# swiss-territorial-data-lab/proj-roadsurf

Hardware: AMD Instinct MI355X
Metric: tiles_per_sec_512x512x3 (higher is better)
Workload: dtype f16 hi + lo operand planes (22 significand bits, 3 MFMA products per product) / f32 accumulate; 1 GPU; Mask R-CNN R50-FPN inference, batch 16 of 512x512 3-band tiles per GPU (BASELINE configs[1]), 800x800 network input; seeded synthetic weights, saturated: 1000 proposals and 100 detections per tile; batch_per_gpu=16, lanes=2, lane_streams=independent, num_classes=2, weights=random

## Files before the change

### include/rs_engine.h

```cpp
#ifndef RS_ENGINE_H
#define RS_ENGINE_H

#include <stddef.h>
#include <stdint.h>

#ifdef __cplusplus
extern "C" {
#endif

#define RS_ABI_VERSION 1
#define RS_SPEC_MAX_LEVELS 5
#define RS_SPEC_MAX_ANCHORS 8
#define RS_NUM_PHASES 3
#define RS_MASK_SIDE 28
#define RS_MAX_CLASSES 80
#define RS_TRAIN_MAX_CLASSES 8

typedef struct rs_spec {
  int32_t struct_size;
  int32_t in_channels;
  int32_t flip_channels;
  float pixel_mean[4];
  float pixel_std[4];
  int32_t min_size_test;
// ... 100 lines not shown
                     const void* w1p, const float* b1, void* t1n, const void* x0, const void* wsc, int n, int h, int w, int width,
                     void* stream);

int rs_op_bneck_tail_split(const void* t1, int64_t t1_lo, const void* w2, const float* s2, const float* b2, const void* w3p, const float* s3,
                           const float* b3, const void* x, int64_t x_lo, void* out, int64_t out_lo, const void* w1p, const float* s1,
                           const float* b1, void* t1n, int64_t t1n_lo, const void* x0, int64_t x0_lo, int n, int h, int w, int width,
                           void* stream);

int rs_op_mask_overlap(const uint8_t* det_masks, int n_det, const uint8_t* label_masks, int n_labels, int h, int w, int32_t* inter,
                       int32_t* label_area, void* stream);
int rs_engine_label_overlap(rs_engine* e, int tile, const uint8_t* label_masks_dev, int n_labels, int32_t* inter_dev, int32_t* label_area_dev);

int rs_op_conv_variant(int m, int cin, int k, int cout, int cin2, int deconv2x, int out_f32, int* stages_out);

int rs_debug_set_conv_probe(void* buffer);

int rs_op_set_saturation_counter(void* dev_u64);

int rs_op_conv2d_split(const void* in, int64_t in_lo, const void* w, int64_t w_lo, const float* wscale, const float* bias, void* out, int64_t out_lo,
                       const void* residual, int64_t res_lo, const void* upsample_add, int64_t up_lo,
                       int n, int hi, int wi, int cin, int in_halo, int kh, int kw, int stride, int pad, int cout, int kpad,
                       int out_halo, int relu, int out_f32, int deconv2x, int variant, void* stream);

int rs_op_conv2d_dual(const void* in, const void* in2, const void* w, const float* bias, void* out,
                      int n, int hi, int wi, int cin, int in_halo, int kh, int kw, int stride, int pad,
                      int h2, int w2, int cin2, int in2_halo, int stride2,
                      int cout, int kpad, int out_halo, int relu, int variant, void* stream);

int rs_op_conv2d_dgrad(const void* dy, const void* w_t, void* dx, const void* res, const float* res32, const void* mask,
                       const void* down, int n, int hi, int wi, int cin, int ho, int wo, int cout, int kh, int kw, int stride,
                       int pad, int kpad, int halo, int variant, void* stream);

int rs_op_conv2d_wgrad(const void* dy, const void* in, float* grad, const float* scale, int n, int hi, int wi, int cin,
                       int in_halo, int kh, int kw, int stride, int pad, int cout, int kpad, int dy_halo, int splits,
                       void* stream);
int rs_op_conv2d_wgrad_f32(const void* dy, const void* in, float* grad, const float* scale, int n, int hi, int wi, int cin,
                       int in_halo, int kh, int kw, int stride, int pad, int cout, int kpad, int dy_halo, int splits,
                       void* stream);

int rs_op_nms(const float* boxes, const int32_t* counts, const uint8_t* valid, uint8_t* keep,
              int segments, int cap, float thresh, void* stream);
int rs_op_batched_nms(const float* boxes, const int32_t* counts, const uint8_t* valid, uint8_t* keep, int images,
                      int segments_per_image, int cap, float thresh, int rule, void* stream);
int rs_op_batched_nms_decision(const float* boxes, const int32_t* counts, const uint8_t* valid, uint8_t* keep, int images,
                               int segments_per_image, int cap, float thresh, int rule, int32_t* rule_out, float* unit_out, void* stream);

// ... 99 lines not shown
```

### proj_roadsurf_amd/csrc/common.h

```cpp
#pragma once
#include <hip/hip_runtime.h>
#include <stdint.h>
#include <stdio.h>

typedef _Float16 half_t;
typedef _Float16 half4 __attribute__((ext_vector_type(4)));
typedef _Float16 half8 __attribute__((ext_vector_type(8)));
typedef float f32x4 __attribute__((ext_vector_type(4)));

#define RS_OK 0
#define RS_ERR_ARG -1
#define RS_ERR_HIP -2
#define RS_ERR_BLOB -3
#define RS_ERR_UNSUPPORTED -4

void rs_set_error(const char* fmt, ...);

#define RS_HIP(expr)                                                                       \
  do {                                                                                     \
    hipError_t _e = (expr);                                                                \
    if (_e != hipSuccess) {                                                                \
      rs_set_error("%s:%d: %s -> %s", __FILE__, __LINE__, #expr, hipGetErrorString(_e));   \
      return RS_ERR_HIP;                                                                   \
    }                                                                                      \
// ... 116 lines not shown
  const half_t* mask;
  int out_stride;
  long long* probe;
  int persist;
  int stages;
  const half_t* head_w;
  const float* head_b;
  float* head_out;
  int nseg;
  int seg_tiles;
  int tail_tiles;
  int split;
  long long in_lo, w_lo, out_lo, res_lo, up_lo, in2_lo;
  const float* wscale;
  long long head_w_lo;
  const float* head_scale;
  ConvSeg seg[RS_MAX_SEGS];
  unsigned long long* sat;
};

int launch_conv(const ConvParams& p, hipStream_t stream, int force_variant , int use_glds);
int conv_choose_variant(ConvParams& p, int force_variant, int use_glds);
extern thread_local int g_last_conv_variant;

struct StemPoolParams {
  const half_t* in;
  const half_t* wf;
  const float* bias;
  half_t* out;
  int N, in_Hp, in_Wp;
  int Hc, Wc;
  int Hq, Wq;
  unsigned long long* sat;
};
int launch_stem_pool(const StemPoolParams& p, hipStream_t stream);
struct StemPoolSplitParams {
  const half_t* in; long long in_lo;
  const half_t* wf;
  const float* wscale;
  const float* bias;
  half_t* out; long long out_lo;
  int N, in_Hp, in_Wp;
  int Hc, Wc;
  int Hq, Wq;
  unsigned long long* sat;
};
// ... 93 lines not shown
```

### proj_roadsurf_amd/csrc/conv_deep.hip

```cpp
#include "common.h"

namespace {

constexpr int BN = 256, NT = 512, MI = 4, WCH = 4;
constexpr int ASTAGE = 256 * 128, WSTAGE = BN * 128;
constexpr int W_BASE = 3 * ASTAGE;
constexpr int LDS_BYTES = 3 * ASTAGE + 2 * WSTAGE;

__device__ __forceinline__ void glds16(const half_t* g, char* lds_wave_base) {
  __builtin_amdgcn_global_load_lds((const __attribute__((address_space(1))) void*)g,
                                   (__attribute__((address_space(3))) void*)lds_wave_base, 16, 0, 0);
}

template <int DBG, bool TRAIN, int NJ, bool SPLIT>
__device__ __forceinline__ void conv_deep_tile(const ConvParams& p, char* smem, const half_t* g_in, const half_t* g_w, const float* g_bias, void* g_out,
                                               float* g_head_out, const int Ho, const int Wo, const int in_Hp, const int in_Wp, const int out_Hp, const int out_Wp,
                                               const int M, const int m0, const int n0, const int q, const long long in_lo, const long long out_lo,
                                               const float* g_wscale) {
  constexpr int APS = (NJ + 1) / 2;
  constexpr int WPX = NJ * 16;
  const int tid = threadIdx.x;
  const int lane = tid & 63;
  const int wave = __builtin_amdgcn_readfirstlane(tid >> 6);
  const int wpx = wave / WCH, wch = wave % WCH;
  (void)q;

  const int lrow = lane >> 3, lchk = lane & 7;
  const half_t* aptr[APS];
  const half_t* wptr[4];
  unsigned aoffb[APS], woffb[4];
#pragma unroll
  for (int ps = 0; ps < APS; ++ps) {
    int m = m0 + ps * 64 + wave * 8 + lrow;
    if (m >= M) m = M - 1;
    const int x = m % Wo;
    const int t = m / Wo;
    const int y = t % Ho;
// ... 270 lines not shown
  }

#ifdef RS_CLOCK_PROBE
  if (p.probe && tid == 0) {
    p.probe[2 * q] = (long long)(__builtin_amdgcn_s_memtime() - pr_t0);
    p.probe[2 * q + 1] = (long long)(__builtin_amdgcn_s_memrealtime() - pr_r0);
  }
#endif
  const int crow = n0 + wch * 64 + fq * 16;
  float bias[16];
#pragma unroll
  for (int i = 0; i < MI; ++i) {
    const f32x4 b4 = *(const f32x4*)(g_bias + crow + i * 4);
    bias[i * 4 + 0] = b4[0]; bias[i * 4 + 1] = b4[1]; bias[i * 4 + 2] = b4[2]; bias[i * 4 + 3] = b4[3];
  }
  float wsc[SPLIT ? 16 : 1];
  if constexpr (SPLIT) {
#pragma unroll
    for (int i = 0; i < MI; ++i) {
      const f32x4 s4 = *(const f32x4*)(g_wscale + crow + i * 4);
      wsc[i * 4 + 0] = s4[0]; wsc[i * 4 + 1] = s4[1]; wsc[i * 4 + 2] = s4[2]; wsc[i * 4 + 3] = s4[3];
    }
  }
  unsigned satc = 0;
  if (!TRAIN && SPLIT && p.head_w) {
    const half_t* hw = p.head_w + (long long)fi * 256 + wch * 64 + fq * 8;
    const half8 ha0 = *(const half8*)hw, ha1 = *(const half8*)(hw + 32);
    const half8 hl0 = *(const half8*)(hw + p.head_w_lo), hl1 = *(const half8*)(hw + p.head_w_lo + 32);
    f32x4 hacc[NJ];
#pragma unroll
    for (int j = 0; j < NJ; ++j) {
      half8 b0, b1, l0, l1;
      const bool mv = m0 + wpx * WPX + j * 16 + fi < M;
      unsigned sath = 0;
#pragma unroll
      for (int i = 0; i < MI; ++i)
#pragma unroll
        for (int r = 0; r < 4; ++r) {
          float f = acc[i][j][r] * wsc[i * 4 + r] + bias[i * 4 + r];
          if (p.relu) f = f > 0.f ? f : 0.f;
          sath += mv ? rs_sat_bad(f) : 0u;
          f = f > 65504.f ? 65504.f : (f < -65504.f ? -65504.f : f);
          const half_t h = (half_t)f;
          const half_t l = (half_t)(f - (float)h);
          if (i < 2) { b0[i * 4 + r] = h; l0[i * 4 + r] = l; } else { b1[(i - 2) * 4 + r] = h; l1[(i - 2) * 4 + r] = l; }
        }
// ... 228 lines not shown
  }
  if (p.nseg) {
    int t0 = 0;
#pragma unroll
    for (int i = 0; i < RS_MAX_SEGS; ++i)
      if (i < p.nseg && L >= p.seg[i].tile0) {
        g_in = p.seg[i].in; g_w = p.seg[i].w; g_bias = p.seg[i].bias; g_out = p.seg[i].out; g_head_out = p.seg[i].head_out;
        Ho = p.seg[i].Ho; Wo = p.seg[i].Wo; in_Hp = p.seg[i].in_Hp; in_Wp = p.seg[i].in_Wp;
        out_Hp = p.seg[i].out_Hp; out_Wp = p.seg[i].out_Wp; M = p.seg[i].M; t0 = p.seg[i].tile0;
        if constexpr (SPLIT) { in_lo = p.seg[i].in_lo; out_lo = p.seg[i].out_lo; g_wscale = p.seg[i].wscale; }
      }
    L -= t0;
  }
  const int n0 = (L % tiles_n) * BN;
  const int m0 = (L / tiles_n) * BM;
  if (half < 0 || NJF != 8) {
    conv_deep_tile<DBG, TRAIN, NJF, SPLIT>(p, smem, g_in, g_w, g_bias, g_out, g_head_out, Ho, Wo, in_Hp, in_Wp, out_Hp, out_Wp, M, m0, n0, q, in_lo, out_lo, g_wscale);
  } else {
    if (m0 + half * (BM / 2) >= M) return;
    conv_deep_tile<DBG, TRAIN, NJF == 8 ? 4 : NJF, SPLIT>(p, smem, g_in, g_w, g_bias, g_out, g_head_out, Ho, Wo, in_Hp, in_Wp, out_Hp, out_Wp, M, m0 + half * (BM / 2), n0, q, in_lo, out_lo, g_wscale);
  }
}

}

int rs_device_cu_count() {
  static int ncu[64] = {0};
  int dev = 0;
  if (hipGetDevice(&dev) != hipSuccess || dev < 0 || dev >= 64) return 256;
  if (!ncu[dev]) {
    int n = 0;
    if (hipDeviceGetAttribute(&n, hipDeviceAttributeMultiprocessorCount, dev) != hipSuccess || n <= 0) n = 256;
    ncu[dev] = n;
  }
  return ncu[dev];
}

static int deep_tail_tiles(long long tiles) {
  const int ncu = rs_device_cu_count();
  if (!rs_debug().deep_tail) return 0;
  const int r = (int)(tiles % ncu);
  return (r > 0 && 2 * r <= ncu) ? r : 0;
}

static int no_scratch(const void* kernel, const char* what) {
  hipFuncAttributes a;
// ... 3 lines not shown
  return RS_OK;
}

template <int NJF>
static int launch_deep_nj(ConvParams& p, hipStream_t stream) {
  static bool done = false;
  if (!done) {
    RS_HIP(hipFuncSetAttribute((const void*)conv_deep_kernel<0, false, NJF>, hipFuncAttributeMaxDynamicSharedMemorySize, LDS_BYTES));
    if constexpr (NJF >= 5) RS_HIP(hipFuncSetAttribute((const void*)conv_deep_kernel<0, false, NJF, true>, hipFuncAttributeMaxDynamicSharedMemorySize, LDS_BYTES));
    { int rc = no_scratch((const void*)conv_deep_kernel<0, false, NJF>, "conv_deep_kernel"); if (rc) return rc; }
    if constexpr (NJF >= 5) { int rc = no_scratch((const void*)conv_deep_kernel<0, false, NJF, true>, "conv_deep_kernel (split operands)"); if (rc) return rc; }
    done = true;
  }
  const long long nblk = (long long)(p.Cout / BN) * cdiv(p.M, 32 * NJF);
  RS_CHECK(nblk < (1ll << 30), RS_ERR_ARG, "conv_deep: grid too large");
  p.tail_tiles = 0;
  if (p.split) {
    if constexpr (NJF >= 5) hipLaunchKernelGGL((conv_deep_kernel<0, false, NJF, true>), dim3((unsigned)nblk), dim3(NT), LDS_BYTES, stream, p);
    else RS_CHECK(false, RS_ERR_UNSUPPORTED, "conv_deep: the split-operand mode has the 160 .. 256-pixel tiles only");
    RS_HIP(hipGetLastError());
    return RS_OK;
  }
  hipLaunchKernelGGL((conv_deep_kernel<0, false, NJF>), dim3((unsigned)nblk), dim3(NT), LDS_BYTES, stream, p);
  RS_HIP(hipGetLastError());
  return RS_OK;
}

int launch_conv_deep(const ConvParams& p0, hipStream_t stream, int tile_px) {
  ConvParams p = p0;
  p.nseg = 0;
  RS_CHECK(p.mode == 0 && !p.in2 && p.Cin % 64 == 0 && p.Cout % BN == 0 && p.M > 0, RS_ERR_ARG,
           "conv_deep: unsupported shape (mode %d, Cin %d, Cout %d)", p.mode, p.Cin, p.Cout);
  RS_CHECK(!p.head_w || (p.Cout == BN && p.head_b && p.head_out && !p.res && !p.up && !p.down && !p.res32 && !p.mask), RS_ERR_ARG,
           "conv_deep: the fused head needs Cout == 256, its bias and output, and no other epilogue option");
  RS_CHECK(p.out_stride <= 1, RS_ERR_UNSUPPORTED, "conv_deep: no strided scatter");
  RS_CHECK(!p.split || (p.wscale && (!p.head_w || p.head_scale) && !p.down && !p.res32 && !p.mask), RS_ERR_UNSUPPORTED, "conv_deep: the split-operand mode needs the row scales (the fused head's too) and has no training epilogue");
  if (p.split) {
    const long long in_px = (long long)cdiv(p.M, p.Ho * p.Wo) * p.in_Hp * p.in_Wp;
    RS_CHECK((p.in_lo + in_px * p.in_Cs) * 2 < (1ll << 32) && (p.w_lo + (long long)p.Cout * p.Kpad) * 2 < (1ll << 32), RS_ERR_UNSUPPORTED,
             "conv_deep: split-operand tensor of more than 4 GB (input %lld elements per plane)", in_px * p.in_Cs);
  }
  if (tile_px != 256) {
    RS_CHECK(tile_px >= 64 && tile_px <= 224 && tile_px % 32 == 0 && !p.down && !p.res32 && !p.mask, RS_ERR_ARG,
             "conv_deep: tile height %d (256, or 64 .. 224 in steps of 32 without training epilogue options)", tile_px);
    switch (tile_px / 32) {
      case 2: return launch_deep_nj<2>(p, stream);
// ... 96 lines not shown
```

### proj_roadsurf_amd/csrc/conv_igemm.hip

```cpp
#include "common.h"

namespace {

template <int WPX, int WCH, int MI, int NJ>
struct Tile {
  static constexpr int NW = WPX * WCH;
  static constexpr int NT = NW * 64;
  static constexpr int BM = WPX * NJ * 16;
  static constexpr int BN = WCH * MI * 16;
  static constexpr int STAGE = (BM + BN) * 128;
  static constexpr int LDS = 2 * STAGE + 1024;
};

__device__ __forceinline__ void glds16(const half_t* g, char* lds_wave_base) {
  __builtin_amdgcn_global_load_lds((const __attribute__((address_space(1))) void*)g,
                                   (__attribute__((address_space(3))) void*)lds_wave_base, 16, 0, 0);
}

template <int WPX, int WCH, int MI, int NJ, bool SMALLC, bool GLDS, bool PERSIST, bool TRAIN = false, bool SPLIT = false>
__global__ __launch_bounds__(WPX* WCH * 64) void conv_igemm_kernel(const ConvParams p) {
  using T = Tile<WPX, WCH, MI, NJ>;
  constexpr int NW = T::NW, BM = T::BM, BN = T::BN;
  constexpr int PA = BM / (NW * 8);
  constexpr int PW = (BN + NW * 8 - 1) / (NW * 8);
// ... 541 lines not shown

int launch_conv(const ConvParams& p_in, hipStream_t stream, int force_variant, int use_glds) {
  if (use_glds < 0) {
    RS_CHECK(!p_in.in2, RS_ERR_UNSUPPORTED, "conv: the fp32 kernel has no second K source");
    g_last_conv_variant = -1;
    return launch_conv_f32(p_in, stream, use_glds == -2, force_variant);
  }
  ConvParams p = p_in;
  const int nk2 = p.in2 ? (p.Cin2 >> 6) : 0;
  const bool train_opts = p.down || p.res32 || p.mask || p.out_stride > 1;
  RS_CHECK(p.M > 0, RS_ERR_ARG, "conv: M=%d", p.M);
  RS_CHECK(p.Kpad % 64 == 0, RS_ERR_ARG, "conv: Kpad %d not a multiple of 64", p.Kpad);
  const bool smallc = p.Cin < 64;
  if (smallc) {
    RS_CHECK((p.Cin == 8 || p.Cin == 4) && p.koff != nullptr, RS_ERR_ARG, "conv: small-Cin path needs Cin 4 or 8 and a koff table");
  } else {
    RS_CHECK(p.Cin % 64 == 0, RS_ERR_ARG, "conv: Cin %d not a multiple of 64", p.Cin);
    RS_CHECK(p.KH * p.KW * p.Cin + nk2 * 64 <= p.Kpad, RS_ERR_ARG, "conv: K exceeds Kpad");
  }
  if (p.in2) RS_CHECK(!smallc && p.mode == 0 && p.Cin2 % 64 == 0 && p.Cin2 > 0 && p.stride2 >= 1, RS_ERR_ARG, "conv: bad second K source (Cin2 %d)", p.Cin2);
  const int rows = p.Cout * (p.mode != 0 ? 4 : 1);
  int v = conv_choose_variant(p, force_variant, use_glds);
  if (v == 22 && p.mode == 2 && !conv_wreg_ok(p)) v = 14;
  RS_CHECK(!(train_opts && (p.mode != 0 || (v == 12 && p.out_stride > 1) || (v >= 15 && v <= 20))), RS_ERR_UNSUPPORTED, "conv: training epilogue options need mode 0 (and no scatter on conv_deep)");
  if (v == 22 || v == 23 || v == 25 || v == 26) {
    RS_CHECK(conv_wreg_ok(p) && !train_opts, RS_ERR_UNSUPPORTED, "conv: variant %d takes 1x1 / Cin 256 / Cout %% 256 == 0 inference layers only", v);
    g_last_conv_variant = v;
    return launch_conv_wreg(p, stream, v == 23 ? 8 : (v == 25 ? 2 : (v == 26 ? 4 : 0)));
  }
  if (v == 12 || (v >= 15 && v <= 20)) {
    RS_CHECK(!p.in2, RS_ERR_UNSUPPORTED, "conv: variant %d has no second K source", v);
    g_last_conv_variant = v;
    return launch_conv_deep(p, stream, v == 12 ? 256 : (v <= 17 ? 160 + 32 * (v - 15) : 64 + 32 * (v - 18)));
  }
  RS_CHECK(!(p.mode != 0 && p.Cout % 128 != 0), RS_ERR_ARG, "deconv needs Cout %% 128 == 0");
  RS_CHECK(!(p.mode == 2 && !(p.dot_w && p.dot_cls && p.dot_slot && p.dot_out && (v == 0 || v == 10 || v == 14))), RS_ERR_ARG, "fused mask predictor needs its pointers and the 128x128, 64x256 or 128x256 tile");
  g_last_conv_variant = smallc ? 5 : v;
  if (smallc) {
    RS_CHECK(v == 1, RS_ERR_ARG, "conv: small-Cin path is built for the 256x64 tile only (Cout=%d)", p.Cout);
    if (rs_debug().stem_small_tile) return launch_variant<4, 1, 4, 2, true, false>(p, stream, use_glds);
    return launch_variant<4, 1, 4, 4, true, false>(p, stream, use_glds);
  }
  switch (v) {
    case 0:
      RS_CHECK(rows % 128 == 0, RS_ERR_ARG, "conv: variant 0 needs Cout %% 128 == 0");
      return launch_variant<2, 2, 4, 4, false, true>(p, stream, use_glds);
    case 1:
      RS_CHECK(rows % 64 == 0, RS_ERR_ARG, "conv: variant 1 needs Cout %% 64 == 0");
      return launch_variant<4, 1, 4, 4, false, true>(p, stream, use_glds);
    case 2:
      RS_CHECK(rows % 16 == 0 && p.out_f32, RS_ERR_ARG, "conv: variant 2 is the 16-channel-tile fp32-out head kernel");
// ... 28 lines not shown
```

### proj_roadsurf_amd/csrc/detect.h

```cpp
#pragma once
#include "common.h"

#define RS_MAX_LEVELS 5
#define RS_MAX_ANCHORS 8

struct RpnParams {
  const float* head[RS_MAX_LEVELS];
  uint32_t* keys[RS_MAX_LEVELS];
  int H[RS_MAX_LEVELS], W[RS_MAX_LEVELS], stride[RS_MAX_LEVELS];
  float base[RS_MAX_LEVELS][RS_MAX_ANCHORS][4];
  float offset;
  int L, A, N, cs;
  int topk;
  float img_h, img_w;
  const float* img_hw;
  float wx, wy, ww, wh, scale_clamp, min_size;
  float* cand_boxes;
  float* cand_scores;
  uint8_t* cand_valid;
  int* cand_count;
  int* cand_index;
  int debug;
  int cand_cap;
};
// ... 79 lines not shown
  int K, cap, dets_per_image;
  float scale_x, scale_y, out_w, out_h;
  float* det_boxes_net;
  float* det_boxes;
  float* det_scores;
  int* det_classes;
  int* det_roi;
  int* det_count;
  unsigned long long* part_keys;
  int* part_count;
};

struct MaskPredictParams {
  const half_t* in;
  const float* w;
  const float* b;
  const int* slot_list;
  const int* det_classes;
  const int* n_entries;
  float* out;
  int S;
  int f32;
  long long in_lo;
};

struct PasteParams {
  const float* probs;
  const float* det_boxes;
  const int* slot_list;
  const int* n_entries;
  uint8_t* out;
  int S, out_h, out_w;
  float threshold;
};

struct CropParams {
  const float* det_boxes;
  const int* det_count;
  const uint8_t* masks;
  int n, D, h, w, Wb;
  int* rects;
  unsigned int* offsets;
  unsigned long long* total;
  uint8_t* data;
};
int launch_mask_crops(const CropParams& p, hipStream_t s);
// ... 13 lines not shown
```

### proj_roadsurf_amd/csrc/detect_kernels.hip

```cpp
#include "detect.h"

namespace {

__device__ __forceinline__ uint32_t fkey(float f) {
  f = f + 0.0f;
  const uint32_t u = __float_as_uint(f);
  return (u & 0x80000000u) ? ~u : (u | 0x80000000u);
}
__device__ __forceinline__ float fkey_inv(uint32_t k) {
  const uint32_t u = (k & 0x80000000u) ? (k & 0x7fffffffu) : ~k;
  return __uint_as_float(u);
}

template <int T>
__device__ void bitonic_sort_desc(unsigned long long* s, int n, int tid) {
  for (int k = 2; k <= n; k <<= 1) {
    for (int j = k >> 1; j > 0; j >>= 1) {
      for (int i = tid; i < n; i += T) {
        const int ixj = i ^ j;
        if (ixj > i) {
          const unsigned long long a = s[i], b = s[ixj];
          const bool desc = (i & k) == 0;
          if (desc ? (a < b) : (a > b)) { s[i] = b; s[ixj] = a; }
        }
// ... 1457 lines not shown
    const half_t* x = p.in + pix * 256 + sub * 16;
    const half8 a = *(const half8*)x, b = *(const half8*)(x + 8);
#pragma unroll
    for (int i = 0; i < 8; ++i) { xv[i] = (float)a[i]; xv[8 + i] = (float)b[i]; }
  }
  float s = 0.f;
#pragma unroll
  for (int i = 0; i < 16; ++i) s += xv[i] * w[i];
  s += __shfl_xor(s, 8, 16);
  s += __shfl_xor(s, 4, 16);
  s += __shfl_xor(s, 2, 16);
  s += __shfl_xor(s, 1, 16);
  if (sub == 0) {
    const float logit = s + p.b[cls];
    const float prob = rs_fdiv(1.f, 1.f + expf(-logit));
    p.out[(long long)slot * SS + (pix - (long long)entry * SS)] = prob;
  }
}

__global__ __launch_bounds__(256) void mask_sigmoid_kernel(const MaskPredictParams p) {
  const int total = *p.n_entries;
  const int SS = p.S * p.S;
  const long long gid = (long long)blockIdx.x * 256 + threadIdx.x;
  if (gid >= (long long)total * SS) return;
  const int entry = (int)(gid / SS);
  const int slot = p.slot_list[entry];
  float* o = p.out + (long long)slot * SS + (gid - (long long)entry * SS);
  const float logit = *o + p.b[p.det_classes[slot]];
  *o = rs_fdiv(1.f, 1.f + expf(-logit));
}

__global__ __launch_bounds__(256) void paste_masks_kernel(const PasteParams p) {
  const int total = *p.n_entries;
  const int Wb = (p.out_w + 7) >> 3;
  const int Ww = (Wb + 3) >> 2;
  const long long gid = (long long)blockIdx.x * 256 + threadIdx.x;
  const long long per = (long long)p.out_h * Ww;
  if (gid >= (long long)total * per) return;
  const int entry = (int)(gid / per);
  const int rem = (int)(gid - (long long)entry * per);
  const int y = rem / Ww, xw = rem - y * Ww;
  const int slot = p.slot_list[entry];
  const float* bx = p.det_boxes + (long long)slot * 4;
  const float x0 = bx[0], y0 = bx[1], x1 = bx[2], y1 = bx[3];
  const float* m = p.probs + (long long)slot * p.S * p.S;
  const int S = p.S;
  unsigned int word = 0;
// ... 273 lines not shown
```

### proj_roadsurf_amd/csrc/engine.hip

```cpp
#include <stdarg.h>
#include <string.h>

#include <cmath>
#include <functional>
#include <map>
#include <set>
#include <string>
#include <vector>

#include "../../include/rs_engine.h"
#include "detect.h"
#include "train.h"

static thread_local char g_err[1024] = "";
static bool g_trainer_unfused_shortcut = false;

static RsDebug g_debug;
static bool g_debug_loaded = false;
void rs_debug_reload() {
  RsDebug d;
  auto rd = [](const char* name, int* v) { const char* e = getenv(name); if (e && *e) *v = atoi(e); };
  rd("RS_CONV_SINGLE_STAGE_NK", &d.conv_single_stage_nk); rd("RS_CONV_PERSIST", &d.conv_persist); rd("RS_CONV_TUNED", &d.conv_tuned);
  rd("RS_CONV_DEEP", &d.conv_deep); rd("RS_CONV_WIDE_PX", &d.conv_wide_px); rd("RS_CONV_WREG", &d.conv_wreg); rd("RS_WREG_DBG", &d.wreg_dbg); rd("RS_ROI_BWD_ATOMIC", &d.roi_bwd_atomic); rd("RS_WREG_WAVES", &d.wreg_waves); rd("RS_STEM_SMALL_TILE", &d.stem_small_tile); rd("RS_DEEP_DBG", &d.deep_dbg);
  rd("RS_DECONV_VARIANT", &d.deconv_variant); rd("RS_FUSE_MASK_PREDICTOR", &d.fuse_mask_predictor); rd("RS_SIDE_STREAM", &d.side_stream);
  rd("RS_NARROW_ROIALIGN", &d.narrow_roialign); rd("RS_USE_GLDS", &d.use_glds); rd("RS_FUSE_SHORTCUT", &d.fuse_shortcut); rd("RS_MERGE_LEVELS", &d.merge_levels); rd("RS_FUSE_RPN_HEADS", &d.fuse_rpn_heads); rd("RS_DEEP_TAIL", &d.deep_tail); rd("RS_DEEP_TILE_PX", &d.deep_tile_px); rd("RS_FUSE_BNECK", &d.fuse_bneck); rd("RS_FUSE_STEM", &d.fuse_stem);
  rd("RS_USE_GRAPH", &d.use_graph); rd("RS_GRAPH_SMALL", &d.graph_small); rd("RS_TRAIN_ROI_SIDE", &d.train_roi_side);
  rd("RS_TRAIN_SIDE", &d.train_side); rd("RS_WGRAD_TARGET", &d.wgrad_target); rd("RS_WGRAD_CB", &d.wgrad_cb);
  rd("RS_SELECT_DEBUG", &d.select_debug); rd("RS_NMS_DEBUG", &d.nms_debug); rd("RS_ROI_WINDOW", &d.roi_window); rd("RS_ROI_ORDER", &d.roi_order);
// ... 1026 lines not shown
    RS_CHECK(dw && db && wrows(dw) == 1024, RS_ERR_BLOB, "deconv weights missing / wrong rows");
    RS_CHECK(pw && pb && pw->dtype == DT_F32, RS_ERR_BLOB, "mask predictor weights missing");
    const bool fuse = f32 ? false : rs_debug().fuse_mask_predictor != 0;
    ConvParams dp;
    memset(&dp, 0, sizeof dp);
    if ((rc = set_split(&dp, "roi_heads.mask_head.deconv", dw, &curm, nullptr, nullptr, nullptr, nullptr))) return rc;
    dp.in = curm.p; dp.w = (const half_t*)dw->dev; dp.bias = (const float*)db->dev;
    dp.Ho = MR; dp.Wo = MR; dp.in_Hp = curm.Hp(); dp.in_Wp = curm.Wp(); dp.in_Cs = 256; dp.in_off = 1; dp.stride = 1; dp.KH = dp.KW = 1;
    dp.Cin = 256; dp.Kpad = (int)dw->dims[1]; dp.Cout = 256; dp.out_Hp = 2 * MR; dp.out_Wp = 2 * MR; dp.out_Cs = 256; dp.out_pad = 0; dp.relu = 1;
    dp.m_count = det_total; dp.m_mul = MR * MR;
    const int per_roi = MR * MR;
    if (fuse) {
      dp.mode = 2; dp.out = nullptr;
      dp.dot_w = (const float*)pw->dev; dp.dot_cls = det_classes; dp.dot_slot = slot_list; dp.dot_out = mask_probs;
      dp.dot_k = (int)pw->dims[0];
      const int glds = use_glds, Dc = D;
      const bool sp = split;
      float* probs = mask_probs;
      const size_t zero_per_tile = (size_t)D * RS_MASK_SIDE * RS_MASK_SIDE * 4;
      Stage st;
      st.name = "mask.deconv_predict";
      st.flops_per_image = 2.0 * D * per_roi * 256 * 1024 + 2.0 * D * RS_MASK_SIDE * RS_MASK_SIDE * 256;
      st.bytes_per_image = (double)D * per_roi * 256 * 2 * (split ? 2 : 1) + (double)D * RS_MASK_SIDE * RS_MASK_SIDE * 4;
      st.fn = [dp, per_roi, Dc, glds, probs, zero_per_tile, sp](int n, hipStream_t s) mutable {
        RS_HIP(hipMemsetAsync(probs, 0, zero_per_tile * n, s));
        dp.M = n * Dc * per_roi;
        const int dv = rs_debug().deconv_variant;
        return launch_conv(dp, s, (dv == 22 && (sp || !(rs_debug().conv_wreg && glds > 0))) ? 14 : dv, glds);
      };
      stages.push_back(st);
      MaskPredictParams mp;
      mp.f32 = 0;
      mp.in = nullptr; mp.w = nullptr; mp.b = (const float*)pb->dev; mp.slot_list = slot_list; mp.det_classes = det_classes;
      mp.n_entries = det_total; mp.out = mask_probs; mp.S = RS_MASK_SIDE;
      Stage st2;
      st2.name = "mask.bias_sigmoid";
      st2.fn = [mp, Dc](int n, hipStream_t s) { return launch_mask_sigmoid(mp, n * Dc, s); };
      stages.push_back(st2);
    } else {
      Act dec;
      if ((rc = new_act(&dec, "mask_deconv", R, 2 * MR, 2 * MR, 256, 0))) return rc;
      dp.mode = 1; dp.out = dec.p; dp.out_lo = dec.lo;
      {
        const int glds = use_glds, Dc = D;
        Stage st;
        st.name = "mask.deconv";
        st.flops_per_image = 2.0 * D * per_roi * 256 * 1024;
        st.bytes_per_image = (double)D * per_roi * 256 * 2 * 5;
        dp.sat = sat_slot();
        st.fn = [dp, per_roi, Dc, glds](int n, hipStream_t s) mutable { dp.M = n * Dc * per_roi; return launch_conv(dp, s, -1, glds); };
        stages.push_back(st);
      }
      MaskPredictParams mp;
      mp.in = dec.p; mp.w = (const float*)pw->dev; mp.b = (const float*)pb->dev; mp.slot_list = slot_list; mp.det_classes = det_classes;
      mp.n_entries = det_total; mp.out = mask_probs; mp.S = RS_MASK_SIDE; mp.f32 = f32 ? 1 : (split ? 2 : 0); mp.in_lo = dec.lo;
      Stage st;
      st.name = "mask.predict_sigmoid";
      st.bytes_per_image = (double)D * RS_MASK_SIDE * RS_MASK_SIDE * (256 * 2 + 4);
      const int Dc = D;
      st.fn = [mp, Dc](int n, hipStream_t s) { return launch_mask_predict(mp, n * Dc, s); };
      stages.push_back(st);
    }
    const int Wb = (tile_w + 7) / 8;
    if ((rc = alloc((void**)&masks, (size_t)R * tile_h * Wb))) return rc;
    reg("masks", masks, DT_U8, {NB, D, tile_h, Wb}, 0);
    if ((rc = alloc((void**)&crop_data, (size_t)R * tile_h * Wb))) return rc;
    if ((rc = alloc((void**)&crop_rects, (size_t)R * 16))) return rc;
    if ((rc = alloc((void**)&crop_offsets, (size_t)R * 4))) return rc;
    if ((rc = alloc((void**)&crop_total, 16))) return rc;
    {
      PasteParams pm;
      pm.probs = mask_probs; pm.det_boxes = det_boxes; pm.slot_list = slot_list; pm.n_entries = det_total; pm.out = masks;
      pm.S = RS_MASK_SIDE; pm.out_h = tile_h; pm.out_w = tile_w; pm.threshold = S.mask_threshold;
      Stage st;
      st.name = "mask.paste";
      st.bytes_per_image = (double)D * tile_h * Wb;
// ... 447 lines not shown
  const Stage& s = e->stages[i];
  if (name_out) { strncpy(name_out, s.name.c_str(), 95); name_out[95] = 0; }
  if (ms_total) *ms_total = s.ms_total;
  if (calls) *calls = s.calls;
  if (flops) *flops = s.last_flops;
  if (bytes) *bytes = s.last_bytes;
  return RS_OK;
}

int rs_engine_stage_kernel(rs_engine* e, int i, char* name_out) {
  RS_CHECK(e && i >= 0 && i < (int)e->stages.size() && name_out, RS_ERR_ARG, "stage index");
  static const char* names[] = {"conv_igemm_kernel<2,2,4,4> 128x128", "conv_igemm_kernel<4,1,4,4> 256x64", "conv_igemm_kernel<4,1,1,4> 256x16 f32-out",
                                "conv_igemm_kernel<4,2,4,4> 256x128", "conv_igemm_kernel<2,4,4,8> 256x256", "conv_igemm_kernel<4,1,4,4,smallC> 256x64 stem",
                                "(retired)",
                                "conv_igemm_kernel<2,2,4,2> 64x128", "conv_igemm_kernel<4,1,4,2> 128x64", "conv_igemm_kernel<2,2,4,1> 32x128",
                                "conv_igemm_kernel<2,4,4,2> 64x256", "(retired)",
                                "conv_deep_kernel 256x256 (3 activation + 2 weight LDS stages)",
                                "bneck_tail_kernel 128 px (conv2 + conv3 + next conv1 chained through registers)",
                                "conv_igemm_kernel<2,4,4,4> 128x256",
                                "conv_deep_kernel 160x256", "conv_deep_kernel 192x256", "conv_deep_kernel 224x256",
                                "conv_deep_kernel 64x256", "conv_deep_kernel 96x256", "conv_deep_kernel 128x256",
                                "stem_pool_kernel (conv 7x7 s2 + ReLU + max-pool 3x3 s2, 8x8 pooled pixels per workgroup)",
                                "conv1x1_wreg_kernel 32 px x 256 ch (persistent, weights in registers, operand tiles by LDS-DMA, two workgroups per CU)",
                                "bneck_tail_split_kernel 128 px (conv2 + conv3 + next conv1 chained through registers)"};
  const int v = e->stages[i].variant;
  const char* s = v == -1 ? "conv_f32_mfma_kernel" : (v >= 0 && v <= 23 ? names[v] : "");
  if (e->split && v >= 0 && v <= 23) {
    snprintf(name_out, 96, "%.62s [split: hi+lo planes, 3 MFMA blocks]", s);
    return RS_OK;
  }
  strncpy(name_out, s, 95);
  name_out[95] = 0;
  return RS_OK;
}

int rs_engine_stage_variant(rs_engine* e, int i) {
  if (!e || i < 0 || i >= (int)e->stages.size()) return -2;
  return e->stages[i].variant;
}

int rs_op_conv_variant(int m, int cin, int k, int cout, int cin2, int deconv2x, int out_f32, int* stages_out) {
  ConvParams p;
  memset(&p, 0, sizeof p);
  p.M = m; p.Cin = cin; p.KH = p.KW = k; p.Cout = cout; p.mode = deconv2x ? 1 : 0; p.out_f32 = out_f32;
  p.stride = 1; p.in_Cs = cin; p.out_Cs = cout;
  p.Kpad = (k * k * (cin < 64 ? 8 : cin) + cin2 + 63) / 64 * 64;
  if (cin < 64 && k == 7) p.Kpad = 256;
  static const half_t dummy = (half_t)0;
  if (cin2 > 0) { p.in2 = &dummy; p.Cin2 = cin2; }
  const int v = conv_choose_variant(p, -1, 1);
// ... 81 lines not shown
  }
  return rc;
}

int rs_debug_set_conv_probe(void* buffer) { g_conv_probe = (long long*)buffer; return RS_OK; }
int rs_op_set_saturation_counter(void* dev_u64) { g_op_sat = (unsigned long long*)dev_u64; return RS_OK; }

int rs_op_conv2d(const void* in, const void* w, const float* bias, void* out, const void* residual, const void* upsample_add,
                 int n, int hi, int wi, int cin, int in_halo, int kh, int kw, int stride, int pad, int cout, int kpad,
                 int out_halo, int relu, int out_f32, int deconv2x, int variant, int use_glds, void* stream) {
  return op_conv2d(in, w, bias, out, residual, upsample_add, n, hi, wi, cin, in_halo, kh, kw, stride, pad, cout, kpad, out_halo,
                   relu, out_f32, deconv2x, variant, use_glds, stream, nullptr, 0, 0, 0, 0, 1);
}

int rs_op_conv2d_split(const void* in, int64_t in_lo, const void* w, int64_t w_lo, const float* wscale, const float* bias, void* out, int64_t out_lo,
                       const void* residual, int64_t res_lo, const void* upsample_add, int64_t up_lo,
                       int n, int hi, int wi, int cin, int in_halo, int kh, int kw, int stride, int pad, int cout, int kpad,
                       int out_halo, int relu, int out_f32, int deconv2x, int variant, void* stream) {
  SplitArgs sa = {in_lo, w_lo, out_lo, res_lo, up_lo, wscale};
  return op_conv2d(in, w, bias, out, residual, upsample_add, n, hi, wi, cin, in_halo, kh, kw, stride, pad, cout, kpad, out_halo,
                   relu, out_f32, deconv2x, variant, 1, stream, nullptr, 0, 0, 0, 0, 1, &sa);
}

int rs_op_conv2d_dual(const void* in, const void* in2, const void* w, const float* bias, void* out,
                      int n, int hi, int wi, int cin, int in_halo, int kh, int kw, int stride, int pad,
                      int h2, int w2, int cin2, int in2_halo, int stride2,
                      int cout, int kpad, int out_halo, int relu, int variant, void* stream) {
  RS_CHECK(in2, RS_ERR_ARG, "null argument");
  return op_conv2d(in, w, bias, out, nullptr, nullptr, n, hi, wi, cin, in_halo, kh, kw, stride, pad, cout, kpad, out_halo,
                   relu, 0, 0, variant, 1, stream, in2, h2, w2, cin2, in2_halo, stride2);
}

int rs_op_bneck_tail(const void* t1, const void* w2, const float* b2, const void* w3p, const float* b3, const void* x, void* out,
                     const void* w1p, const float* b1, void* t1n, const void* x0, const void* wsc, int n, int h, int w, int width, void* stream) {
  RS_CHECK(t1 && w2 && b2 && w3p && b3 && out && n > 0 && h > 0 && w > 0, RS_ERR_ARG, "bad argument");
  RS_CHECK(width == 64 || width == 128, RS_ERR_UNSUPPORTED, "bneck_tail: bottleneck width %d (64 or 128)", width);
  BneckParams p;
  memset(&p, 0, sizeof p);
  p.t1 = (const half_t*)t1; p.w2 = (const half_t*)w2; p.b2 = b2; p.w3p = (const half_t*)w3p; p.b3 = b3; p.x = (const half_t*)x; p.out = (half_t*)out;
  p.w1p = (const half_t*)w1p; p.b1 = b1; p.t1n = (half_t*)t1n; p.x0 = (const half_t*)x0; p.wsc = (const half_t*)wsc;
  p.M = n * h * w; p.H = h; p.W = w; p.Hp = h + 2; p.Wp = w + 2; p.CB = width / 64;
  p.sat = g_op_sat;
  return launch_bneck_tail(p, (hipStream_t)stream);
}

int rs_op_bneck_tail_split(const void* t1, int64_t t1_lo, const void* w2, const float* s2, const float* b2, const void* w3p, const float* s3, const float* b3,
// ... 281 lines not shown
```

### proj_roadsurf_amd/engine.py

```python
from __future__ import annotations

import ctypes as C
import weakref
import math
import os
import time
from typing import Any, Dict, Iterator, List, Optional, Sequence, Tuple

import numpy as np

from .spec import BATCHED_NMS_MODES, EngineSpec
from .weights import pack_weights

_LIB: Optional[C.CDLL] = None
LIB_PATH = os.environ.get("RS_ENGINE_LIB") or os.path.join(os.path.dirname(os.path.abspath(__file__)), "librs_engine.so")
MAX_LEVELS, MAX_ANCHORS, MASK_SIDE = 5, 8, 28
DT_NP = {1: np.float16, 2: np.float32, 3: np.int32, 4: np.uint8, 5: np.float16}
DT_SPLIT16 = 5


class RsError(RuntimeError):
    pass


# ... 80 lines not shown
    lib.rs_engine_fetch_crops_async.argtypes = [vp, i32, C.POINTER(RsDets), C.POINTER(RsMaskCrops)]
    lib.rs_engine_fetch_crops_wait.argtypes = [vp, C.POINTER(RsMaskCrops)]
    lib.rs_engine_fetch.argtypes = [vp, i32, C.POINTER(RsDets)]
    lib.rs_engine_stream.argtypes = [vp]
    lib.rs_engine_stream.restype = vp
    lib.rs_engine_set_profiling.argtypes = [vp, i32]
    lib.rs_debug_run_stages_matching.argtypes = [vp, C.c_char_p, i32]
    lib.rs_engine_stage_count.argtypes = [vp]
    lib.rs_engine_saturation.argtypes = [vp, C.POINTER(C.c_int64), i32]
    lib.rs_op_set_saturation_counter.argtypes = [vp]
    lib.rs_engine_stage_info.argtypes = [vp, i32, C.c_char_p, C.POINTER(C.c_double), i32p, C.POINTER(C.c_double), C.POINTER(C.c_double)]
    lib.rs_engine_stage_kernel.argtypes = [vp, i32, C.c_char_p]
    lib.rs_engine_stage_variant.argtypes = [vp, i32]
    lib.rs_op_conv_variant.argtypes = [i32] * 7 + [i32p]
    lib.rs_engine_tensor.argtypes = [vp, C.c_char_p, C.POINTER(vp), i32p, i32p, C.POINTER(C.c_int64), i32p]
    lib.rs_engine_tensor_count.argtypes = [vp]
    lib.rs_engine_tensor_name.argtypes = [vp, i32, C.c_char_p]
    lib.rs_engine_net_shape.argtypes = [vp, i32p, i32p, i32p, i32p]
    lib.rs_op_conv2d.argtypes = [vp, vp, vp, vp, vp, vp] + [i32] * 17 + [vp]
    lib.rs_op_bneck_tail.argtypes = [vp] * 12 + [i32, i32, i32, i32, vp]
    lib.rs_op_conv2d_dual.argtypes = [vp, vp, vp, vp, vp] + [i32] * 19 + [vp]
    i64 = C.c_int64
    lib.rs_op_conv2d_split.argtypes = [vp, i64, vp, i64, vp, vp, vp, i64, vp, i64, vp, i64] + [i32] * 16 + [vp]
    lib.rs_op_bneck_tail_split.argtypes = [vp, i64, vp, vp, vp, vp, vp, vp, vp, i64, vp, i64, vp, vp, vp, vp, i64, vp, i64, i32, i32, i32, i32, vp]
    lib.rs_op_conv2d_dgrad.argtypes = [vp] * 7 + [i32] * 14 + [vp]
    lib.rs_op_conv2d_wgrad.argtypes = [vp, vp, vp, vp] + [i32] * 13 + [vp]
    lib.rs_op_nms.argtypes = [vp, vp, vp, vp, i32, i32, C.c_float, vp]
    lib.rs_op_batched_nms.argtypes = [vp, vp, vp, vp, i32, i32, i32, C.c_float, i32, vp]
    lib.rs_op_batched_nms_decision.argtypes = [vp, vp, vp, vp, i32, i32, i32, C.c_float, i32, vp, vp, vp]
    lib.rs_op_det_merge.argtypes = [vp] * 5 + [i32] * 4 + [C.c_float] * 4 + [vp] * 7
    lib.rs_spec_batched_nms.argtypes = [C.POINTER(RsSpec)]
    lib.rs_op_roi_align.argtypes = [C.POINTER(vp), i32p, i32p, f32p, i32, vp, i32, i32, i32, i32, vp, vp, vp]
    lib.rs_op_roi_align_bwd.argtypes = [C.POINTER(vp), i32p, i32p, f32p, i32, vp, i32, i32, i32, i32, vp, vp]
    f32 = C.c_float
    lib.rs_op_match.argtypes = [vp, i32, vp, vp, vp, vp, vp, vp, i32, i32, i32, f32, f32, i32, i32, i32, i32, vp]
    lib.rs_op_subsample.argtypes = [vp, vp, vp, i32, i32, i32, f32, i32, i32, C.c_uint32, vp]
    lib.rs_op_rpn_loss.argtypes = [vp] * 6 + [i32] * 6 + [f32, f32, vp]
    lib.rs_op_box_loss.argtypes = [vp] * 6 + [i32, i32, i32, f32, f32p, f32, vp]
    lib.rs_op_mask_loss.argtypes = [vp] * 5 + [i32, i32, i32, f32, vp]
    lib.rs_op_sgd_momentum.argtypes = [vp, vp, vp, C.c_int64, f32, f32, f32, f32, i32, vp]
    lib.rs_op_fold_weights.argtypes = [vp] * 4 + [i32] * 6 + [vp]
    lib.rs_resize_shape.argtypes = [i32, i32, i32, i32, i32p, i32p]
    lib.rs_resize_shape.restype = None
    lib.rs_resize_coeffs.argtypes = [i32, i32, i32p, i32p]
    i64p, f64p = C.POINTER(C.c_int64), C.POINTER(C.c_double)
    lib.rs_vectorize_masks.argtypes = [vp, i32, i32, i32, C.c_double, i32]
# ... 1041 lines not shown
```

Measured before the change: 918.1 tiles/s.

## Fuse split-operand mask deconv with per-class predictor dot in conv_deep kernel

Adds a DOT path to the conv_deep tile that applies scale, bias and ReLU to the deconv accumulators, dots them with the selected class's predictor weights, reduces across waves in LDS, and writes mask logits straight to their 2x-upsampled positions. This variant is now the default for the split-precision mask deconv. It also drops the full memset of the logits buffer; the sigmoid kernel instead zeroes only the unused detection slots. The intent is to avoid the slower variant-14 path plus the separate predictor pass and memset, at the cost of an extra LDS reduction and a barrier in the epilogue.

```diff
diff --git a/include/rs_engine.h b/include/rs_engine.h
--- a/include/rs_engine.h
+++ b/include/rs_engine.h
@@ -146,6 +146,10 @@
                        int n, int hi, int wi, int cin, int in_halo, int kh, int kw, int stride, int pad, int cout, int kpad,
                        int out_halo, int relu, int out_f32, int deconv2x, int variant, void* stream);
 
+int rs_op_deconv_predict_split(const void* in, int64_t in_lo, const void* w, int64_t w_lo, const float* wscale, const float* bias, const float* dot_w,
+                               int dot_k, const int* dot_cls, const int* dot_slot, const int* m_count, float* logits, int slots, int n, int h, int wd,
+                               int cin, int in_halo, int kpad, int variant, void* stream);
+
 int rs_op_conv2d_dual(const void* in, const void* in2, const void* w, const float* bias, void* out,
                       int n, int hi, int wi, int cin, int in_halo, int kh, int kw, int stride, int pad,
                       int h2, int w2, int cin2, int in2_halo, int stride2,
diff --git a/proj_roadsurf_amd/csrc/common.h b/proj_roadsurf_amd/csrc/common.h
--- a/proj_roadsurf_amd/csrc/common.h
+++ b/proj_roadsurf_amd/csrc/common.h
@@ -162,6 +162,8 @@
 int launch_conv(const ConvParams& p, hipStream_t stream, int force_variant , int use_glds);
 int conv_choose_variant(ConvParams& p, int force_variant, int use_glds);
 extern thread_local int g_last_conv_variant;
+bool conv_deep_dot_ok(const ConvParams& p);
+int launch_conv_deep_dot(const ConvParams& p, hipStream_t stream);
 
 struct StemPoolParams {
   const half_t* in;
diff --git a/proj_roadsurf_amd/csrc/conv_deep.hip b/proj_roadsurf_amd/csrc/conv_deep.hip
--- a/proj_roadsurf_amd/csrc/conv_deep.hip
+++ b/proj_roadsurf_amd/csrc/conv_deep.hip
@@ -12,7 +12,7 @@
                                    (__attribute__((address_space(3))) void*)lds_wave_base, 16, 0, 0);
 }
 
-template <int DBG, bool TRAIN, int NJ, bool SPLIT>
+template <int DBG, bool TRAIN, int NJ, bool SPLIT, bool DOT = false>
 __device__ __forceinline__ void conv_deep_tile(const ConvParams& p, char* smem, const half_t* g_in, const half_t* g_w, const float* g_bias, void* g_out,
                                                float* g_head_out, const int Ho, const int Wo, const int in_Hp, const int in_Wp, const int out_Hp, const int out_Wp,
                                                const int M, const int m0, const int n0, const int q, const long long in_lo, const long long out_lo,
@@ -329,6 +329,53 @@
       wsc[i * 4 + 0] = s4[0]; wsc[i * 4 + 1] = s4[1]; wsc[i * 4 + 2] = s4[2]; wsc[i * 4 + 3] = s4[3];
     }
   }
+  if constexpr (DOT) {
+    const int cb = wch * 64 + fq * 16;
+    const int g = n0 / BN;
+    const int HW = Ho * Wo;
+    float dotp[NJ];
+#pragma unroll
+    for (int j = 0; j < NJ; ++j) {
+      int m = m0 + wpx * WPX + j * 16 + fi;
+      if (m >= M) m = M - 1;
+      const int slot = p.dot_slot[m / HW];
+      const float* wv = p.dot_w + (long long)p.dot_cls[slot] * BN + cb;
+      float sdot = 0.f;
+#pragma unroll
+      for (int i = 0; i < MI; ++i) {
+        const f32x4 w4 = *(const f32x4*)(wv + i * 4);
+#pragma unroll
+        for (int r = 0; r < 4; ++r) {
+          float v = acc[i][j][r] * wsc[i * 4 + r] + bias[i * 4 + r];
+          if (p.relu) v = v > 0.f ? v : 0.f;
+          sdot += v * w4[r];
+        }
+      }
+      sdot += __shfl_xor(sdot, 16);
+      sdot += __shfl_xor(sdot, 32);
+      dotp[j] = sdot;
+    }
+    asm volatile("s_barrier" ::: "memory");
+    float* red = (float*)smem;
+    if (wch > 0 && fq == 0) {
+#pragma unroll
+      for (int j = 0; j < NJ; ++j) red[(((wch - 1) * 2 + wpx) * NJ + j) * 16 + fi] = dotp[j];
+    }
+    __syncthreads();
+    if (wch == 0 && fq == 0) {
+#pragma unroll
+      for (int j = 0; j < NJ; ++j) {
+        float v0 = dotp[j];
+#pragma unroll
+        for (int c = 1; c < WCH; ++c) v0 += red[(((c - 1) * 2 + wpx) * NJ + j) * 16 + fi];
+        const int m = m0 + wpx * WPX + j * 16 + fi;
+        if (m >= M) continue;
+        const int x = m % Wo, t = m / Wo, y = t % Ho, n = t / Ho;
+        p.dot_out[(long long)p.dot_slot[n] * (4 * HW) + (long long)(2 * y + (g >> 1)) * (2 * Wo) + 2 * x + (g & 1)] = v0;
+      }
+    }
+    return;
+  }
   unsigned satc = 0;
   if (!TRAIN && SPLIT && p.head_w) {
     const half_t* hw = p.head_w + (long long)fi * 256 + wch * 64 + fq * 8;
@@ -603,6 +650,23 @@
   }
 }
 
+__global__ __launch_bounds__(NT) void conv_deep_dot_kernel(const ConvParams p) {
+  extern __shared__ __attribute__((aligned(16))) char smem[];
+  int M = p.M;
+  if (p.m_count) {
+    long long mc = (long long)(*p.m_count) * p.m_mul;
+    if (mc < M) M = (int)mc;
+  }
+  const int tiles_n = p.Cout / BN;
+  const int ntiles = tiles_n * ((M + 255) / 256);
+  const int q = blockIdx.x;
+  if (q >= ntiles) return;
+  const int qn = ntiles >> 3, r = ntiles & 7, x = q & 7;
+  const int L = (x < r ? x * (qn + 1) : r * (qn + 1) + (x - r) * qn) + (q >> 3);
+  conv_deep_tile<0, false, 8, true, true>(p, smem, p.in, p.w, p.bias, nullptr, nullptr, p.Ho, p.Wo, p.in_Hp, p.in_Wp, p.out_Hp, p.out_Wp, M, (L / tiles_n) * 256,
+                                          (L % tiles_n) * BN, q, p.in_lo, p.out_lo, p.wscale);
+}
+
 }
 
 int rs_device_cu_count() {
@@ -652,6 +716,33 @@
     return RS_OK;
   }
   hipLaunchKernelGGL((conv_deep_kernel<0, false, NJF>), dim3((unsigned)nblk), dim3(NT), LDS_BYTES, stream, p);
+  RS_HIP(hipGetLastError());
+  return RS_OK;
+}
+
+bool conv_deep_dot_ok(const ConvParams& p) {
+  if (!(p.mode == 2 && p.split && p.wscale && p.Cout == BN && p.Cin > 0 && p.Cin % 64 == 0 && p.KH == 1 && p.KW == 1 && p.stride == 1 && p.M > 0 && p.Ho > 0 && p.Wo > 0 &&
+        !p.in2 && !p.res && !p.up && !p.head_w && !p.down && !p.res32 && !p.mask && p.out_stride <= 1 && p.dot_w && p.dot_cls && p.dot_slot && p.dot_out && p.dot_k > 0))
+    return false;
+  const long long in_px = (long long)cdiv(p.M, p.Ho * p.Wo) * p.in_Hp * p.in_Wp;
+  return (p.in_lo + in_px * p.in_Cs) * 2 < (1ll << 32) && (p.w_lo + 4ll * BN * p.Kpad) * 2 < (1ll << 32) && 4ll * cdiv(p.M, 256) < (1ll << 30);
+}
+
+int launch_conv_deep_dot(const ConvParams& p0, hipStream_t stream) {
+  RS_CHECK(conv_deep_dot_ok(p0), RS_ERR_UNSUPPORTED, "conv_deep: the fused mask predictor takes the split-operand 1x1 deconv groups of 256 channels with both planes within 4 GB (mode %d, Cin %d, Cout %d)",
+           p0.mode, p0.Cin, p0.Cout);
+  static bool done = false;
+  if (!done) {
+    RS_HIP(hipFuncSetAttribute((const void*)conv_deep_dot_kernel, hipFuncAttributeMaxDynamicSharedMemorySize, LDS_BYTES));
+    { int rc = no_scratch((const void*)conv_deep_dot_kernel, "conv_deep_dot_kernel"); if (rc) return rc; }
+    done = true;
+  }
+  ConvParams p = p0;
+  p.nseg = 0;
+  p.tail_tiles = 0;
+  p.Cout = 4 * BN;
+  const long long nblk = 4ll * cdiv(p.M, 256);
+  hipLaunchKernelGGL(conv_deep_dot_kernel, dim3((unsigned)nblk), dim3(NT), LDS_BYTES, stream, p);
   RS_HIP(hipGetLastError());
   return RS_OK;
 }
diff --git a/proj_roadsurf_amd/csrc/conv_igemm.hip b/proj_roadsurf_amd/csrc/conv_igemm.hip
--- a/proj_roadsurf_amd/csrc/conv_igemm.hip
+++ b/proj_roadsurf_amd/csrc/conv_igemm.hip
@@ -587,11 +587,17 @@
   const int rows = p.Cout * (p.mode != 0 ? 4 : 1);
   int v = conv_choose_variant(p, force_variant, use_glds);
   if (v == 22 && p.mode == 2 && !conv_wreg_ok(p)) v = 14;
+  if (v == 24 && p.mode == 2 && !(use_glds > 0 && conv_deep_dot_ok(p))) v = 14;
   RS_CHECK(!(train_opts && (p.mode != 0 || (v == 12 && p.out_stride > 1) || (v >= 15 && v <= 20))), RS_ERR_UNSUPPORTED, "conv: training epilogue options need mode 0 (and no scatter on conv_deep)");
   if (v == 22 || v == 23 || v == 25 || v == 26) {
     RS_CHECK(conv_wreg_ok(p) && !train_opts, RS_ERR_UNSUPPORTED, "conv: variant %d takes 1x1 / Cin 256 / Cout %% 256 == 0 inference layers only", v);
     g_last_conv_variant = v;
     return launch_conv_wreg(p, stream, v == 23 ? 8 : (v == 25 ? 2 : (v == 26 ? 4 : 0)));
+  }
+  if (v == 24) {
+    RS_CHECK(p.mode == 2, RS_ERR_UNSUPPORTED, "conv: variant 24 is the fused deconv + mask predictor (mode 2) only");
+    g_last_conv_variant = v;
+    return launch_conv_deep_dot(p, stream);
   }
   if (v == 12 || (v >= 15 && v <= 20)) {
     RS_CHECK(!p.in2, RS_ERR_UNSUPPORTED, "conv: variant %d has no second K source", v);
diff --git a/proj_roadsurf_amd/csrc/detect.h b/proj_roadsurf_amd/csrc/detect.h
--- a/proj_roadsurf_amd/csrc/detect.h
+++ b/proj_roadsurf_amd/csrc/detect.h
@@ -125,6 +125,8 @@
   int S;
   int f32;
   long long in_lo;
+  const int* rest_count;
+  int rest_n, rest_d;
 };
 
 struct PasteParams {
diff --git a/proj_roadsurf_amd/csrc/detect_kernels.hip b/proj_roadsurf_amd/csrc/detect_kernels.hip
--- a/proj_roadsurf_amd/csrc/detect_kernels.hip
+++ b/proj_roadsurf_amd/csrc/detect_kernels.hip
@@ -1503,7 +1503,17 @@
   const int total = *p.n_entries;
   const int SS = p.S * p.S;
   const long long gid = (long long)blockIdx.x * 256 + threadIdx.x;
-  if (gid >= (long long)total * SS) return;
+  if (gid >= (long long)total * SS) {
+    if (!p.rest_count) return;
+    const long long sg = gid - (long long)total * SS;
+    long long e = sg / SS;
+    for (int i = 0; i < p.rest_n; ++i) {
+      const int c = p.rest_count[i];
+      if (e < p.rest_d - c) { p.out[((long long)i * p.rest_d + c + e) * SS + (sg - (sg / SS) * SS)] = 0.f; return; }
+      e -= p.rest_d - c;
+    }
+    return;
+  }
   const int entry = (int)(gid / SS);
   const int slot = p.slot_list[entry];
   float* o = p.out + (long long)slot * SS + (gid - (long long)entry * SS);
diff --git a/proj_roadsurf_amd/csrc/engine.hip b/proj_roadsurf_amd/csrc/engine.hip
--- a/proj_roadsurf_amd/csrc/engine.hip
+++ b/proj_roadsurf_amd/csrc/engine.hip
@@ -4,6 +4,7 @@
 #include <cmath>
 #include <functional>
 #include <map>
+#include <memory>
 #include <set>
 #include <string>
 #include <vector>
@@ -1076,20 +1077,31 @@
       st.name = "mask.deconv_predict";
       st.flops_per_image = 2.0 * D * per_roi * 256 * 1024 + 2.0 * D * RS_MASK_SIDE * RS_MASK_SIDE * 256;
       st.bytes_per_image = (double)D * per_roi * 256 * 2 * (split ? 2 : 1) + (double)D * RS_MASK_SIDE * RS_MASK_SIDE * 4;
-      st.fn = [dp, per_roi, Dc, glds, probs, zero_per_tile, sp](int n, hipStream_t s) mutable {
-        RS_HIP(hipMemsetAsync(probs, 0, zero_per_tile * n, s));
+      std::shared_ptr<int> stored = std::make_shared<int>(0);
+      st.fn = [dp, per_roi, Dc, glds, probs, zero_per_tile, sp, stored](int n, hipStream_t s) mutable {
         dp.M = n * Dc * per_roi;
-        const int dv = rs_debug().deconv_variant;
-        return launch_conv(dp, s, (dv == 22 && (sp || !(rs_debug().conv_wreg && glds > 0))) ? 14 : dv, glds);
+        int dv = rs_debug().deconv_variant;
+        if (dv == 22 && sp) dv = rs_debug().conv_deep ? 24 : 14;
+        if (dv == 24 && !(glds > 0 && conv_deep_dot_ok(dp))) dv = 14;
+        if (dv == 22 && !(rs_debug().conv_wreg && glds > 0)) dv = 14;
+        *stored = dv == 24;
+        if (dv != 24) RS_HIP(hipMemsetAsync(probs, 0, zero_per_tile * n, s));
+        return launch_conv(dp, s, dv, glds);
       };
       stages.push_back(st);
       MaskPredictParams mp;
       mp.f32 = 0;
+      mp.rest_count = nullptr; mp.rest_n = 0; mp.rest_d = D;
       mp.in = nullptr; mp.w = nullptr; mp.b = (const float*)pb->dev; mp.slot_list = slot_list; mp.det_classes = det_classes;
       mp.n_entries = det_total; mp.out = mask_probs; mp.S = RS_MASK_SIDE;
       Stage st2;
       st2.name = "mask.bias_sigmoid";
-      st2.fn = [mp, Dc](int n, hipStream_t s) { return launch_mask_sigmoid(mp, n * Dc, s); };
+      const int* dcount = det_count;
+      st2.fn = [mp, Dc, stored, dcount](int n, hipStream_t s) mutable {
+        mp.rest_count = *stored ? dcount : nullptr;
+        mp.rest_n = n;
+        return launch_mask_sigmoid(mp, n * Dc, s);
+      };
       stages.push_back(st2);
     } else {
       Act dec;
@@ -1106,6 +1118,7 @@
         stages.push_back(st);
       }
       MaskPredictParams mp;
+      mp.rest_count = nullptr; mp.rest_n = 0; mp.rest_d = 0;
       mp.in = dec.p; mp.w = (const float*)pw->dev; mp.b = (const float*)pb->dev; mp.slot_list = slot_list; mp.det_classes = det_classes;
       mp.n_entries = det_total; mp.out = mask_probs; mp.S = RS_MASK_SIDE; mp.f32 = f32 ? 1 : (split ? 2 : 0); mp.in_lo = dec.lo;
       Stage st;
@@ -1599,10 +1612,11 @@
                                 "conv_deep_kernel 64x256", "conv_deep_kernel 96x256", "conv_deep_kernel 128x256",
                                 "stem_pool_kernel (conv 7x7 s2 + ReLU + max-pool 3x3 s2, 8x8 pooled pixels per workgroup)",
                                 "conv1x1_wreg_kernel 32 px x 256 ch (persistent, weights in registers, operand tiles by LDS-DMA, two workgroups per CU)",
-                                "bneck_tail_split_kernel 128 px (conv2 + conv3 + next conv1 chained through registers)"};
+                                "bneck_tail_split_kernel 128 px (conv2 + conv3 + next conv1 chained through registers)",
+                                "conv_deep_dot_kernel 256 px x (dy, dx) group"};
   const int v = e->stages[i].variant;
-  const char* s = v == -1 ? "conv_f32_mfma_kernel" : (v >= 0 && v <= 23 ? names[v] : "");
-  if (e->split && v >= 0 && v <= 23) {
+  const char* s = v == -1 ? "conv_f32_mfma_kernel" : (v >= 0 && v <= 24 ? names[v] : "");
+  if (e->split && v >= 0 && v <= 24) {
     snprintf(name_out, 96, "%.62s [split: hi+lo planes, 3 MFMA blocks]", s);
     return RS_OK;
   }
@@ -1730,6 +1744,26 @@
                    relu, out_f32, deconv2x, variant, 1, stream, nullptr, 0, 0, 0, 0, 1, &sa);
 }
 
+int rs_op_deconv_predict_split(const void* in, int64_t in_lo, const void* w, int64_t w_lo, const float* wscale, const float* bias, const float* dot_w, int dot_k,
+                               const int* dot_cls, const int* dot_slot, const int* m_count, float* logits, int slots, int n, int h, int wd, int cin, int in_halo,
+                               int kpad, int variant, void* stream) {
+  RS_CHECK(in && w && wscale && bias && dot_w && dot_cls && dot_slot && logits && n > 0 && h > 0 && wd > 0 && slots > 0 && dot_k > 0 && in_halo >= 0, RS_ERR_ARG, "bad argument");
+  RS_CHECK(variant == 0 || variant == 10 || variant == 14 || variant == 24, RS_ERR_ARG, "deconv_predict: variant %d (0, 10, 14 or 24)", variant);
+  ConvParams p;
+  memset(&p, 0, sizeof p);
+  p.in = (const half_t*)in; p.w = (const half_t*)w; p.bias = bias;
+  p.M = n * h * wd; p.Ho = h; p.Wo = wd;
+  p.in_Hp = h + 2 * in_halo; p.in_Wp = wd + 2 * in_halo; p.in_Cs = cin; p.in_off = in_halo;
+  p.stride = 1; p.KH = p.KW = 1; p.Cin = cin; p.Kpad = kpad; p.Cout = 256;
+  p.out_Hp = 2 * h; p.out_Wp = 2 * wd; p.out_Cs = 256; p.relu = 1; p.mode = 2;
+  p.m_count = m_count; p.m_mul = h * wd;
+  p.dot_w = dot_w; p.dot_cls = dot_cls; p.dot_slot = dot_slot; p.dot_out = logits; p.dot_k = dot_k;
+  p.split = 1; p.in_lo = in_lo; p.w_lo = w_lo; p.wscale = wscale;
+  if (variant == 24) RS_CHECK(conv_deep_dot_ok(p), RS_ERR_UNSUPPORTED, "deconv_predict: variant 24 does not take this layer (launch_conv would run it on variant 14)");
+  else RS_HIP(hipMemsetAsync(logits, 0, (size_t)slots * 4 * h * wd * sizeof(float), (hipStream_t)stream));
+  return launch_conv(p, (hipStream_t)stream, variant, 1);
+}
+
 int rs_op_conv2d_dual(const void* in, const void* in2, const void* w, const float* bias, void* out,
                       int n, int hi, int wi, int cin, int in_halo, int kh, int kw, int stride, int pad,
                       int h2, int w2, int cin2, int in2_halo, int stride2,
diff --git a/proj_roadsurf_amd/engine.py b/proj_roadsurf_amd/engine.py
--- a/proj_roadsurf_amd/engine.py
+++ b/proj_roadsurf_amd/engine.py
@@ -126,6 +126,7 @@
     lib.rs_op_conv2d_dual.argtypes = [vp, vp, vp, vp, vp] + [i32] * 19 + [vp]
     i64 = C.c_int64
     lib.rs_op_conv2d_split.argtypes = [vp, i64, vp, i64, vp, vp, vp, i64, vp, i64, vp, i64] + [i32] * 16 + [vp]
+    lib.rs_op_deconv_predict_split.argtypes = [vp, i64, vp, i64, vp, vp, vp, i32, vp, vp, vp, vp] + [i32] * 8 + [vp]
     lib.rs_op_bneck_tail_split.argtypes = [vp, i64, vp, vp, vp, vp, vp, vp, vp, i64, vp, i64, vp, vp, vp, vp, i64, vp, i64, i32, i32, i32, i32, vp]
     lib.rs_op_conv2d_dgrad.argtypes = [vp] * 7 + [i32] * 14 + [vp]
     lib.rs_op_conv2d_wgrad.argtypes = [vp, vp, vp, vp] + [i32] * 13 + [vp]
```

Result: no change. 916.6 tiles/s (-0.2%).
